# lrm2017/Fastest_Image_Pattern_Matching

Hardware: AMD Instinct MI355X
Metric: template matches/sec + ms/search, 4024×3036 src ±180°; HBM GB/s vs roofline (higher is better)
Workload: dtype u8

## Files before the change

### fastest_image_pattern_matching_amd/csrc/fpm_kernels.hip

```cpp
#include <float.h>
#include <stdio.h>
#include <stdlib.h>
#include <limits.h>

#include <map>
#include <mutex>
#include <type_traits>
#include <utility>

#include "fpm_kernels.h"
#include "fpm_rrect.h"

static void ensure_lds_attr(const void* fn, size_t bytes) {
    if (bytes <= 65536) return;
    int dev = 0;
    (void)hipGetDevice(&dev);
    static std::mutex mu;
    static std::map<std::pair<int, const void*>, size_t> done;
    std::lock_guard<std::mutex> lock(mu);
    size_t& cur = done[std::make_pair(dev, fn)];
    if (bytes <= cur) return;
    (void)hipFuncSetAttribute(fn, hipFuncAttributeMaxDynamicSharedMemorySize, (int)bytes);
    cur = bytes;
}
// ... 2523 lines not shown
                        } else {
                            pk = bilerp_row4(v, fxv, fyv);
                        }
                    }
                    if (ABL == 4 ? pk == 0x9e3779b9u && c0 < 0 : ry0 + lr + 8 * i <= ry1)
                        st_at<uint32_t>(tile, st_lane + 256u * i, (pk & colmask) ^ kRoiFlip);
                }
                continue;
            }
#pragma unroll
            for (int i = 0; i < 4; ++i) {
                if (ry0 + lr + 8 * i > ry1) break;
                uint32_t pk = 0;
#pragma unroll
                for (int u = 0; u < 4; ++u) {
                    const int X = (int)(X0r[i] + adv[u]) >> kTapShift;
                    const int Y = (int)(Y0r[i] + bdv[u]) >> kTapShift;
                    int v;
                    if (in_lds) {
                        const int sx = sat_s16(X >> kInterBits), sy = sat_s16(Y >> kInterBits);
                        const int fx = X & (kInterTab - 1), fy = Y & (kInterTab - 1);
                        const uint8_t* p = FT + (sy - by0) * ftw + (sx - bxa);
                        int v0, v1, v2, v3;
                        if ((unsigned)sx < (unsigned)(W - 1) && (unsigned)sy < (unsigned)(H - 1)) {
                            v0 = p[0]; v1 = p[1]; v2 = p[ftw]; v3 = p[ftw + 1];
                        } else if (sx >= W || sx + 1 < 0 || sy >= H || sy + 1 < 0) {
                            v0 = v1 = v2 = v3 = 0;
                        } else {
                            const bool x0 = sx >= 0 && sx < W, x1 = sx + 1 >= 0 && sx + 1 < W;
                            const bool y0 = sy >= 0 && sy < H, y1 = sy + 1 >= 0 && sy + 1 < H;
                            v0 = x0 && y0 ? p[0] : 0;
                            v1 = x1 && y0 ? p[1] : 0;
                            v2 = x0 && y1 ? p[ftw] : 0;
                            v3 = x1 && y1 ? p[ftw + 1] : 0;
                        }
                        const int h0 = 32 * v0 + fx * (v1 - v0), h1 = 32 * v2 + fx * (v3 - v2);
                        v = (32 * h0 + fy * (h1 - h0) + 512) >> 10;
                    } else {
                        v = roi_tap(lvl, W, H, a.P, X, Y);
                    }
                    if (c0 + u >= RW) v = 0;
                    pk |= (uint32_t)v << (8 * u);
                }
                st_at<uint32_t>(tile, st_lane + 256u * i, pk ^ kRoiFlip);
            }
        }
    }
}

typedef int fpm_v4i __attribute__((ext_vector_type(4)));
constexpr int kBandRows = 2 * kMmaRows;
constexpr int kBandSrc = kBandRows + 6;
constexpr int kStageRows = (kBandSrc + 3) / 4;
constexpr int kStageBatch = 5;

__device__ __forceinline__ uint32_t wave_sum_u32(uint32_t v) {
#pragma unroll
    for (int m = 32; m >= 1; m >>= 1) v += (uint32_t)__shfl_xor((int)v, m, 64);
    return v;
}

__device__ __forceinline__ uint32_t funnel(uint32_t hi, uint32_t lo, int sh) {
    return sh == 0 ? lo : __builtin_amdgcn_alignbyte(hi, lo, sh);
}

__device__ __forceinline__ void band_mfma(const uint8_t* ap, const uint8_t* bp, int nk, fpm_v4i acc[7]) {
    fpm_v4i c0 = {0, 0, 0, 0}, c1 = c0, c2 = c0, c3 = c0, c4 = c0, c5 = c0, c6 = c0;
    for (int k = 0; k < nk; ++k) {
        const fpm_v4i av = *(const fpm_v4i*)__builtin_assume_aligned(ap + 64 * k, 16);
        const uint8_t* bk = (const uint8_t*)__builtin_assume_aligned(bp + 64 * k, 16);
        const uint4 lo = *(const uint4*)bk;
        const uint2 hi = *(const uint2*)(bk + 16);
        const uint32_t w0 = lo.x, w1 = lo.y, w2 = lo.z, w3 = lo.w, w4 = hi.x, w5 = hi.y;
        const uint32_t a10 = __builtin_amdgcn_alignbyte(w1, w0, 1), a21 = __builtin_amdgcn_alignbyte(w2, w1, 1),
                       a32 = __builtin_amdgcn_alignbyte(w3, w2, 1), a43 = __builtin_amdgcn_alignbyte(w4, w3, 1),
                       a54 = __builtin_amdgcn_alignbyte(w5, w4, 1);
        const uint32_t b10 = __builtin_amdgcn_alignbyte(w1, w0, 2), b21 = __builtin_amdgcn_alignbyte(w2, w1, 2),
                       b32 = __builtin_amdgcn_alignbyte(w3, w2, 2), b43 = __builtin_amdgcn_alignbyte(w4, w3, 2),
                       b54 = __builtin_amdgcn_alignbyte(w5, w4, 2);
        const uint32_t e10 = __builtin_amdgcn_alignbyte(w1, w0, 3), e21 = __builtin_amdgcn_alignbyte(w2, w1, 3),
                       e32 = __builtin_amdgcn_alignbyte(w3, w2, 3), e43 = __builtin_amdgcn_alignbyte(w4, w3, 3);
        c0 = __builtin_amdgcn_mfma_i32_16x16x64_i8(av, fpm_v4i{(int)w0, (int)w1, (int)w2, (int)w3}, c0, 0, 0, 0);
        c1 = __builtin_amdgcn_mfma_i32_16x16x64_i8(av, fpm_v4i{(int)a10, (int)a21, (int)a32, (int)a43}, c1, 0, 0, 0);
        c2 = __builtin_amdgcn_mfma_i32_16x16x64_i8(av, fpm_v4i{(int)b10, (int)b21, (int)b32, (int)b43}, c2, 0, 0, 0);
        c3 = __builtin_amdgcn_mfma_i32_16x16x64_i8(av, fpm_v4i{(int)e10, (int)e21, (int)e32, (int)e43}, c3, 0, 0, 0);
        c4 = __builtin_amdgcn_mfma_i32_16x16x64_i8(av, fpm_v4i{(int)w1, (int)w2, (int)w3, (int)w4}, c4, 0, 0, 0);
        c5 = __builtin_amdgcn_mfma_i32_16x16x64_i8(av, fpm_v4i{(int)a21, (int)a32, (int)a43, (int)a54}, c5, 0, 0, 0);
        c6 = __builtin_amdgcn_mfma_i32_16x16x64_i8(av, fpm_v4i{(int)b21, (int)b32, (int)b43, (int)b54}, c6, 0, 0, 0);
    }
    acc[0] = c0; acc[1] = c1; acc[2] = c2; acc[3] = c3; acc[4] = c4; acc[5] = c5; acc[6] = c6;
}

__device__ __forceinline__ void band_mfma_ga(const int8_t* ap, const uint8_t* bp, int nk, fpm_v4i acc[7]) {
    fpm_v4i c0 = {0, 0, 0, 0}, c1 = c0, c2 = c0, c3 = c0, c4 = c0, c5 = c0, c6 = c0;
    fpm_v4i p0 = *(const fpm_v4i*)ap, p1 = *(const fpm_v4i*)(ap + 64);
    for (int k = 0; k < nk; ++k) {
        const fpm_v4i av = p0;
        p0 = p1;
        p1 = *(const fpm_v4i*)(ap + 64 * (k + 2));
        asm volatile("" ::: "memory");
        const uint8_t* bk = (const uint8_t*)__builtin_assume_aligned(bp + 64 * k, 16);
        const uint4 lo = *(const uint4*)bk;
        const uint2 hi = *(const uint2*)(bk + 16);
        const uint32_t w0 = lo.x, w1 = lo.y, w2 = lo.z, w3 = lo.w, w4 = hi.x, w5 = hi.y;
        const uint32_t a10 = __builtin_amdgcn_alignbyte(w1, w0, 1), a21 = __builtin_amdgcn_alignbyte(w2, w1, 1),
                       a32 = __builtin_amdgcn_alignbyte(w3, w2, 1), a43 = __builtin_amdgcn_alignbyte(w4, w3, 1),
                       a54 = __builtin_amdgcn_alignbyte(w5, w4, 1);
        const uint32_t b10 = __builtin_amdgcn_alignbyte(w1, w0, 2), b21 = __builtin_amdgcn_alignbyte(w2, w1, 2),
                       b32 = __builtin_amdgcn_alignbyte(w3, w2, 2), b43 = __builtin_amdgcn_alignbyte(w4, w3, 2),
                       b54 = __builtin_amdgcn_alignbyte(w5, w4, 2);
        const uint32_t e10 = __builtin_amdgcn_alignbyte(w1, w0, 3), e21 = __builtin_amdgcn_alignbyte(w2, w1, 3),
                       e32 = __builtin_amdgcn_alignbyte(w3, w2, 3), e43 = __builtin_amdgcn_alignbyte(w4, w3, 3);
        c0 = __builtin_amdgcn_mfma_i32_16x16x64_i8(av, fpm_v4i{(int)w0, (int)w1, (int)w2, (int)w3}, c0, 0, 0, 0);
        c1 = __builtin_amdgcn_mfma_i32_16x16x64_i8(av, fpm_v4i{(int)a10, (int)a21, (int)a32, (int)a43}, c1, 0, 0, 0);
        c2 = __builtin_amdgcn_mfma_i32_16x16x64_i8(av, fpm_v4i{(int)b10, (int)b21, (int)b32, (int)b43}, c2, 0, 0, 0);
        c3 = __builtin_amdgcn_mfma_i32_16x16x64_i8(av, fpm_v4i{(int)e10, (int)e21, (int)e32, (int)e43}, c3, 0, 0, 0);
        c4 = __builtin_amdgcn_mfma_i32_16x16x64_i8(av, fpm_v4i{(int)w1, (int)w2, (int)w3, (int)w4}, c4, 0, 0, 0);
        c5 = __builtin_amdgcn_mfma_i32_16x16x64_i8(av, fpm_v4i{(int)a21, (int)a32, (int)a43, (int)a54}, c5, 0, 0, 0);
        c6 = __builtin_amdgcn_mfma_i32_16x16x64_i8(av, fpm_v4i{(int)b21, (int)b32, (int)b43, (int)b54}, c6, 0, 0, 0);
    }
    acc[0] = c0; acc[1] = c1; acc[2] = c2; acc[3] = c3; acc[4] = c4; acc[5] = c5; acc[6] = c6;
}

template <int NK>
__device__ __forceinline__ void band_mfma_regs(const fpm_v4i* A, const uint8_t* bp, int nk, fpm_v4i acc[7]) {
    fpm_v4i c0 = {0, 0, 0, 0}, c1 = c0, c2 = c0, c3 = c0, c4 = c0, c5 = c0, c6 = c0;
#pragma unroll
    for (int k = 0; k < NK; ++k) {
        if (k >= nk) continue;
        const fpm_v4i av = A[k];
        const uint8_t* bk = (const uint8_t*)__builtin_assume_aligned(bp + 64 * k, 16);
        const uint4 lo = *(const uint4*)bk;
        const uint2 hi = *(const uint2*)(bk + 16);
        const uint32_t w0 = lo.x, w1 = lo.y, w2 = lo.z, w3 = lo.w, w4 = hi.x, w5 = hi.y;
        const uint32_t a10 = __builtin_amdgcn_alignbyte(w1, w0, 1), a21 = __builtin_amdgcn_alignbyte(w2, w1, 1),
                       a32 = __builtin_amdgcn_alignbyte(w3, w2, 1), a43 = __builtin_amdgcn_alignbyte(w4, w3, 1),
                       a54 = __builtin_amdgcn_alignbyte(w5, w4, 1);
        const uint32_t b10 = __builtin_amdgcn_alignbyte(w1, w0, 2), b21 = __builtin_amdgcn_alignbyte(w2, w1, 2),
                       b32 = __builtin_amdgcn_alignbyte(w3, w2, 2), b43 = __builtin_amdgcn_alignbyte(w4, w3, 2),
                       b54 = __builtin_amdgcn_alignbyte(w5, w4, 2);
        const uint32_t e10 = __builtin_amdgcn_alignbyte(w1, w0, 3), e21 = __builtin_amdgcn_alignbyte(w2, w1, 3),
                       e32 = __builtin_amdgcn_alignbyte(w3, w2, 3), e43 = __builtin_amdgcn_alignbyte(w4, w3, 3);
        c0 = __builtin_amdgcn_mfma_i32_16x16x64_i8(av, fpm_v4i{(int)w0, (int)w1, (int)w2, (int)w3}, c0, 0, 0, 0);
        c1 = __builtin_amdgcn_mfma_i32_16x16x64_i8(av, fpm_v4i{(int)a10, (int)a21, (int)a32, (int)a43}, c1, 0, 0, 0);
        c2 = __builtin_amdgcn_mfma_i32_16x16x64_i8(av, fpm_v4i{(int)b10, (int)b21, (int)b32, (int)b43}, c2, 0, 0, 0);
        c3 = __builtin_amdgcn_mfma_i32_16x16x64_i8(av, fpm_v4i{(int)e10, (int)e21, (int)e32, (int)e43}, c3, 0, 0, 0);
        c4 = __builtin_amdgcn_mfma_i32_16x16x64_i8(av, fpm_v4i{(int)w1, (int)w2, (int)w3, (int)w4}, c4, 0, 0, 0);
        c5 = __builtin_amdgcn_mfma_i32_16x16x64_i8(av, fpm_v4i{(int)a21, (int)a32, (int)a43, (int)a54}, c5, 0, 0, 0);
        c6 = __builtin_amdgcn_mfma_i32_16x16x64_i8(av, fpm_v4i{(int)b21, (int)b32, (int)b43, (int)b54}, c6, 0, 0, 0);
    }
    acc[0] = c0; acc[1] = c1; acc[2] = c2; acc[3] = c3; acc[4] = c4; acc[5] = c5; acc[6] = c6;
}

#ifndef FPM_CORR_PRIO
#define FPM_CORR_PRIO 1
#endif
template <int MODE, bool GA, int WPE, int NK = 0, bool PFR = true, int RS = 1, bool SE = false, bool DMA = false,
          bool DB = false>
__global__ __launch_bounds__(256) __attribute__((amdgpu_waves_per_eu(WPE))) void k_roi_corr(RoiArgs a) {
    static_assert(!DMA || (NK > 0 && !PFR), "LDS-DMA staging replaces the register staging of the register-A form");
    static_assert(!DB || DMA, "the double buffer is filled by LDS-DMA");
    static_assert(NK == 0 || (GA && MODE != 3), "the register-A form stages no template rows");
    static_assert(!SE || NK > 0, "the staged epilogue is flushed in the register-A form's staging phase");
    extern __shared__ __attribute__((aligned(16))) uint8_t smem[];
    const int tw = a.tw, th = a.th, RW = tw + 6;
    const int SBp = a.roi_pitch;
    const int TBp = tmpl_lds_pitch(a.tp8);
    uint8_t* const SB0 = smem;
    uint8_t* SB = SB0;
    uint8_t* TB = SB + (size_t)kBandSrc * SBp;
    uint32_t* rall = (uint32_t*)(TB + (GA ? 0 : (size_t)kBandRows * TBp));
    uint32_t* rallq = rall + kBandSrc;
    uint32_t* wi = rallq + kBandSrc;
    uint32_t* wq = wi + kBandSrc * 7;
    uint32_t* lts = wq + kBandSrc * 7;
    uint32_t* rsb = lts + 2 * kMmaRows;
    uint8_t* const SB1 = (uint8_t*)(((uintptr_t)(rsb + 2 * kMmaRows * 49) + 64 + 15) & ~(uintptr_t)15);
    const int tid = threadIdx.x, lane = tid & 63, wv = tid >> 6;
    const int nband = (th + kBandRows - 1) / kBandRows;
    const int rois = roi_count(a), items = rois * nband;
    const int q4 = SBp >> 4;
    const int nwr = (RW + 3) >> 2;
    const int g = lane >> 4, n = lane & 15;
    const int mt = wv & 1, nt = mt + (wv >> 1);
    const int txn = (RW + ROI_T - 1) / ROI_T;
    const XcdSplit xs = xcd_split(items);
    int it_lo = xs.lo + xs.k, it_hi = xs.hi, it_step = xs.nk;
    if (NK > 0) {
        const int64_t span = xs.hi - xs.lo;
        it_lo = xs.lo + (int)(span * xs.k / xs.nk);
        it_hi = xs.lo + (int)(span * (xs.k + 1) / xs.nk);
        it_step = 1;
    }
    constexpr int NA = NK > 0 ? NK : 1;
    fpm_v4i Areg[NA];
#pragma unroll
    for (int k = 0; k < NA; ++k) Areg[k] = fpm_v4i{0, 0, 0, 0};
    int a_band = -1;
    uint4 pv[kStageRows];
    const int lc = min(lane, 2 * txn - 1);
    auto load_rows = [&](int it) {
        const int bd = it / rois, sl = it - bd * rois;
        const int T0n = bd * kBandRows, nsn = min(kBandRows, th - T0n) + 6;
        const uint8_t* rsrc = a.roi + (size_t)sl * a.roi_stride;
        const int wvu = __builtin_amdgcn_readfirstlane(wv);
        int lcv = lc;
        asm volatile("" : "+v"(lcv));
        const uint32_t lane_off = ((uint32_t)(lcv >> 1) << 10) + 16u * (uint32_t)(lcv & 1);
#pragma unroll
        for (int i = 0; i < kStageRows; ++i) {
            const int R = T0n + min(wvu + 4 * i, nsn - 1);
            pv[i] = *(const uint4*)(rsrc + ((size_t)((R >> 5) * txn) << 10) + (R & 31) * ROI_T + lane_off);
        }
    };
    if (NK > 0 && PFR && it_lo < it_hi) load_rows(it_lo);
    int pv_slot = -1, pv_T0 = 0, pv_rb = 0;
    auto flush = [&]() {
        if (!SE || pv_slot < 0) return;
        uint32_t* dst = a.rowsum + (((size_t)th * 49 + 3) & ~(size_t)3) * pv_slot + (size_t)pv_T0 * 49;
        const int nw = pv_rb * 49, n16 = nw >> 2;
        for (int i = tid; i < n16; i += 256) *(uint4*)(dst + 4 * i) = *(const uint4*)(rsb + 4 * i);
        if (tid < (nw & 3)) dst[4 * n16 + tid] = rsb[4 * n16 + tid];
    };
    auto dma_rows = [&](int it, uint8_t* buf) {
        const int bd = it / rois, sl = it - bd * rois;
        const int T0n = bd * kBandRows, nsn = min(kBandRows, th - T0n) + 6;
        const uint8_t* rsrc = a.roi + (size_t)sl * a.roi_stride;
        const uint32_t lane_off = ((uint32_t)(lane >> 1) << 10) + 16u * (uint32_t)(lane & 1);
        const int wvu = __builtin_amdgcn_readfirstlane(wv);
        const bool in_roi = lane < 2 * txn;
#pragma unroll
        for (int i = 0; i < kStageRows; ++i) {
            const int r = wvu + 4 * i;
            if (r < nsn && in_roi) {
                const int R = T0n + r;
                const uint8_t* gp = rsrc + ((size_t)((R >> 5) * txn) << 10) + (R & 31) * ROI_T + lane_off;
                const uint32_t ldsa = __builtin_amdgcn_readfirstlane(lds_offset_of(buf + (size_t)r * SBp));
                uint32_t keep;
                asm volatile("s_mov_b32 %0, m0\n\ts_mov_b32 m0, %2\n\ts_nop 0\n\tglobal_load_lds_dwordx4 %1, off\n\t"
                             "s_mov_b32 m0, %0"
                             : "=&s"(keep) : "v"(gp), "s"(ldsa) : "memory");
            }
        }
    };
    for (int item = it_lo; item < it_hi; item += it_step) {
        int slot, band;
        if (NK > 0) { band = item / rois; slot = item - band * rois; }
        else { slot = item / nband; band = item - slot * nband; }
        SB = DB && ((item - it_lo) & 1) ? SB1 : SB0;
        const int T0 = band * kBandRows, rb = min(kBandRows, th - T0), nsrc = rb + 6;
        __syncthreads();
        if (RS == 0 && tid < kBandSrc) { rall[tid] = 0; rallq[tid] = 0; }
        if (NK > 0) {
            const bool in_roi = lane < 2 * txn;
            if (DB) {
                if (item == it_lo) dma_rows(item, SB);
                asm volatile("s_waitcnt vmcnt(0)" ::: "memory");
                flush();
            } else if (DMA) {
                dma_rows(item, SB);
                flush();
                asm volatile("s_waitcnt vmcnt(0)" ::: "memory");
            } else {
            if (!PFR) load_rows(item);
            flush();
#pragma unroll
            for (int i = 0; i < kStageRows; ++i) {
                const int r = wv + 4 * i;
                if (r < nsrc && lane < q4)
                    *(uint4*)(SB + (size_t)r * SBp + 16 * lane) = in_roi ? pv[i] : make_uint4(kRoiFlip, kRoiFlip, kRoiFlip, kRoiFlip);
            }
            }
            if (band != a_band) {
                a_band = band;
                if (tid < kBandRows) lts[tid] = tid < rb ? (uint32_t)a.tsum[T0 + tid] : 0u;
                if (kMmaRows * mt < rb) {
                    const int8_t* ap = a.tmpl8 + (size_t)(T0 + kMmaRows * mt + n) * a.tp8 + 16 * g;
#pragma unroll
                    for (int k = 0; k < NA; ++k)
                        if (k < a.nk) Areg[k] = *(const fpm_v4i*)(ap + 64 * k);
                }
            }
            if (PFR && item + 1 < it_hi) load_rows(item + 1);
        } else if (MODE != 3) {
            if (tid < kBandRows) lts[tid] = tid < rb ? (uint32_t)a.tsum[T0 + tid] : 0u;
            const uint8_t* rsrc = a.roi + (size_t)slot * a.roi_stride;
            for (int c0 = 0; c0 < q4; c0 += 64) {
                const int c = c0 + lane;
                for (int i0 = 0; i0 < kStageRows; i0 += kStageBatch) {
                    uint4 v[kStageBatch];
#pragma unroll
                    for (int i = 0; i < kStageBatch; ++i) {
                        const int r = wv + 4 * (i0 + i);
                        const int R = T0 + r;
                        v[i] = (r < nsrc && c < 2 * txn)
                                   ? *(const uint4*)(rsrc + ((size_t)((R >> 5) * txn + (c >> 1)) << 10) + (R & 31) * ROI_T + 16 * (c & 1))
                                   : make_uint4(kRoiFlip, kRoiFlip, kRoiFlip, kRoiFlip);
                    }
#pragma unroll
                    for (int i = 0; i < kStageBatch; ++i) {
                        const int r = wv + 4 * (i0 + i);
                        if (r < nsrc && c < q4) *(uint4*)(SB + (size_t)r * SBp + 16 * c) = v[i];
                    }
                }
            }
        }
        __syncthreads();
        if (DB && item + 1 < it_hi) dma_rows(item + 1, SB == SB0 ? SB1 : SB0);
        if (RS >= 1 && MODE != 7 && tid < 4 * nsrc) {
            const int r = tid >> 2, qq = tid & 3;
            const int per = (nwr + 3) >> 2, k0 = qq * per, k1 = min(nwr, k0 + per);
            const uint32_t* row = (const uint32_t*)(SB + (size_t)r * SBp);
            uint32_t s1 = 0, s2 = 0;
            int k = k0;
            for (; k + 8 <= k1; k += 8) {
                uint32_t x[8];
#pragma unroll
                for (int u = 0; u < 8; ++u) x[u] = row[k + u] ^ 0x80808080u;
#pragma unroll
                for (int u = 0; u < 8; ++u) {
                    s1 = __builtin_amdgcn_udot4(x[u], 0x01010101u, s1, false);
                    s2 = __builtin_amdgcn_udot4(x[u], x[u], s2, false);
                }
            }
            for (; k < k1; ++k) {
                const uint32_t x = row[k] ^ 0x80808080u;
                s1 = __builtin_amdgcn_udot4(x, 0x01010101u, s1, false);
                s2 = __builtin_amdgcn_udot4(x, x, s2, false);
            }
            const uint32_t l0 = row[0] ^ 0x80808080u, l1 = row[1] ^ 0x80808080u;
            const int wr = tw >> 2;
            const uint32_t x0 = row[wr], x1 = row[wr + 1], x2 = row[wr + 2];
            const uint32_t e0 = __builtin_amdgcn_alignbyte(x1, x0, (uint32_t)tw) ^ 0x80808080u;
            const uint32_t e1 = __builtin_amdgcn_alignbyte(x2, x1, (uint32_t)tw) ^ 0x80808080u;
            s1 += (uint32_t)__builtin_amdgcn_mov_dpp((int)s1, 0xB1, 0xF, 0xF, false);
            s2 += (uint32_t)__builtin_amdgcn_mov_dpp((int)s2, 0xB1, 0xF, 0xF, false);
            s1 += (uint32_t)__builtin_amdgcn_mov_dpp((int)s1, 0x4E, 0xF, 0xF, false);
            s2 += (uint32_t)__builtin_amdgcn_mov_dpp((int)s2, 0x4E, 0xF, 0xF, false);
#pragma unroll
            for (int h = 0; h < 2; ++h) {
                const int dx = qq + 4 * h;
                if (dx < 7) {
                    const uint32_t ml0 = dx >= 4 ? 0xffffffffu : (1u << (8 * dx)) - 1u;
                    const uint32_t ml1 = dx <= 4 ? 0u : (1u << (8 * (dx - 4))) - 1u;
                    const uint32_t mr0 = dx >= 4 ? 0u : ~((1u << (8 * dx)) - 1u);
                    const uint32_t mr1 = dx <= 4 ? 0xffffu : dx == 5 ? 0xff00u : 0u;
                    const uint32_t a0 = l0 & ml0, a1 = l1 & ml1, b0 = e0 & mr0, b1 = e1 & mr1;
                    uint32_t q1 = __builtin_amdgcn_udot4(a0, 0x01010101u, 0u, false);
                    q1 = __builtin_amdgcn_udot4(a1, 0x01010101u, q1, false);
                    q1 = __builtin_amdgcn_udot4(b0, 0x01010101u, q1, false);
                    q1 = __builtin_amdgcn_udot4(b1, 0x01010101u, q1, false);
                    uint32_t q2 = __builtin_amdgcn_udot4(a0, a0, 0u, false);
                    q2 = __builtin_amdgcn_udot4(a1, a1, q2, false);
                    q2 = __builtin_amdgcn_udot4(b0, b0, q2, false);
                    q2 = __builtin_amdgcn_udot4(b1, b1, q2, false);
                    wi[r * 7 + dx] = s1 - q1;
                    wq[r * 7 + dx] = s2 - q2;
                }
            }
        }
        if (RS == 0 && MODE != 7 && tid < 4 * nsrc) {
            const int r = tid >> 2, qq = tid & 3;
            const int per = (nwr + 3) >> 2, k0 = qq * per, k1 = min(nwr, k0 + per);
            const uint32_t* row = (const uint32_t*)(SB + (size_t)r * SBp);
            uint32_t s1 = 0, s2 = 0;
            int k = k0;
            for (; k + 8 <= k1; k += 8) {
                uint32_t x[8];
#pragma unroll
                for (int u = 0; u < 8; ++u) x[u] = row[k + u] ^ 0x80808080u;
#pragma unroll
                for (int u = 0; u < 8; ++u) {
                    s1 = __builtin_amdgcn_udot4(x[u], 0x01010101u, s1, false);
                    s2 = __builtin_amdgcn_udot4(x[u], x[u], s2, false);
                }
            }
            for (; k < k1; ++k) {
                const uint32_t x = row[k] ^ 0x80808080u;
                s1 = __builtin_amdgcn_udot4(x, 0x01010101u, s1, false);
                s2 = __builtin_amdgcn_udot4(x, x, s2, false);
            }
            atomicAdd(&rall[r], s1);
            atomicAdd(&rallq[r], s2);
        }
        if (!GA) {
            const int trows = (rb + kMmaRows - 1) / kMmaRows * kMmaRows;
            stage_block16(TB, TBp, (const uint8_t*)a.tmpl8 + (size_t)T0 * a.tp8, a.tp8, trows, a.tp8 >> 4, tid, 256);
        }
        if (RS == 0) __syncthreads();
        for (int i = tid; RS == 0 && MODE != 4 && i < nsrc * 7; i += 256) {
            const int r = i / 7, dx = i - r * 7;
            const uint8_t* sbr = SB + (size_t)r * SBp;
            uint32_t q1 = rall[r], q2 = rallq[r];
            for (int c = 0; c < dx; ++c) { const uint32_t v = sbr[c] ^ 0x80u; q1 -= v; q2 -= v * v; }
            for (int c = dx + tw; c < RW; ++c) { const uint32_t v = sbr[c] ^ 0x80u; q1 -= v; q2 -= v * v; }
            wi[i] = q1;
            wq[i] = q2;
        }
        __syncthreads();
        auto partials = [&]() {
            if (MODE == 6 || tid >= 4 * 49) return;
            const int pr = tid >> 1, half = tid & 1;
            const int h = pr / 49, k = pr - h * 49;
            const int chunk = (T0 >> 4) + h;
            const int tlo = kMmaRows * h, thi = min(tlo + kMmaRows, rb);
            const bool ok = chunk < a.nchunk && tlo < thi;
            const int pdy = k / 7, ddx = k - pdy * 7;
            const int t0 = tlo + 8 * half, n8 = ok ? min(8, thi - t0) : 0;
            uint32_t s1 = 0, x[8], y[8];
#pragma unroll
            for (int u = 0; u < 8; ++u) {
                const int i = (t0 + u + pdy) * 7 + ddx;
                x[u] = u < n8 ? wi[i] : 0u;
                y[u] = u < n8 ? wq[i] : 0u;
            }
            uint64_t s2 = 0;
#pragma unroll
            for (int u = 0; u < 8; ++u) { s1 += x[u]; s2 += y[u]; }
            s1 += (uint32_t)__builtin_amdgcn_mov_dpp((int)s1, 0xB1, 0xF, 0xF, false);
            const uint32_t lo = (uint32_t)s2, hi = (uint32_t)(s2 >> 32);
            s2 += (uint64_t)(uint32_t)__builtin_amdgcn_mov_dpp((int)lo, 0xB1, 0xF, 0xF, false) |
                  ((uint64_t)(uint32_t)__builtin_amdgcn_mov_dpp((int)hi, 0xB1, 0xF, 0xF, false) << 32);
            if (ok && half == 0) {
                uint32_t kk = (uint32_t)k;
                asm volatile("" : "+v"(kk));
                const uint32_t wo = ((uint32_t)slot * (uint32_t)a.nchunk + (uint32_t)chunk) * 49u + kk;
                a.wsum[wo] = s1;
                a.wsq[wo] = s2;
            }
        };
        if (RS == 2) partials();
        const bool active = kMmaRows * mt < rb && kMmaRows * nt < nsrc;
        if (FPM_CORR_PRIO == 1) __builtin_amdgcn_s_setprio(1);
        if (MODE != 2 && active) {
            int sr = kMmaRows * nt + n;
            if (sr >= nsrc) sr = 0;
            const uint8_t* bp = SB + (size_t)sr * SBp + 16 * g;
            fpm_v4i acc[7];
            if (FPM_CORR_PRIO == 2) __builtin_amdgcn_s_setprio(1);
            if (NK > 0)
                band_mfma_regs<NA>(Areg, bp, a.nk, acc);
            else if (GA)
                band_mfma_ga(a.tmpl8 + (size_t)(T0 + kMmaRows * mt + n) * a.tp8 + 16 * g, bp, a.nk, acc);
            else
                band_mfma(TB + (size_t)(kMmaRows * mt + n) * TBp + 16 * g, bp, a.nk, acc);
            if (FPM_CORR_PRIO == 2) __builtin_amdgcn_s_setprio(0);
            uint32_t* rs_out = a.rowsum + (((size_t)th * 49 + 3) & ~(size_t)3) * slot + (size_t)T0 * 49;
            const uint32_t kFix = 16384u * (uint32_t)tw;
            int t0 = kMmaRows * mt + 4 * g;
            asm volatile("" : "+v"(t0));
            const int s_ = kMmaRows * nt + n;
            const uint4 ts4 = *(const uint4*)(lts + t0);
#pragma unroll
            for (int r = 0; r < 4; ++r) {
                const int t = t0 + r, dy = s_ - t;
                if (t < rb && s_ < nsrc && dy >= 0 && dy < 7) {
                    const uint32_t ts = r == 0 ? ts4.x : r == 1 ? ts4.y : r == 2 ? ts4.z : ts4.w;
                    if (MODE == 5) {
                        uint32_t x = ts;
#pragma unroll
                        for (int d = 0; d < 7; ++d) x += (uint32_t)acc[d][r];
                        if (x == 0x9e3779b9u && a.W < 0) rs_out[t] = x;
                        continue;
                    }
                    const uint32_t o = (uint32_t)(t * 49 + dy * 7);
                    if (SE) {
#pragma unroll
                        for (int d = 0; d < 7; ++d) rsb[o + d] = (uint32_t)acc[d][r] + 128u * (wi[s_ * 7 + d] + ts) - kFix;
                        continue;
                    }
#pragma unroll
                    for (int d = 0; d < 7; ++d) rs_out[o + d] = (uint32_t)acc[d][r] + 128u * (wi[s_ * 7 + d] + ts) - kFix;
                }
            }
        }
        if (FPM_CORR_PRIO == 1) __builtin_amdgcn_s_setprio(0);
        if (RS == 1) partials();
        if (RS == 0 && MODE != 6 && tid < 2 * 49) {
            const int h = tid / 49, k = tid - h * 49;
            const int chunk = (T0 >> 4) + h;
            const int tlo = kMmaRows * h, thi = min(tlo + kMmaRows, rb);
            if (chunk < a.nchunk && tlo < thi) {
                const int pdy = k / 7, ddx = k - pdy * 7;
                uint32_t s1 = 0;
                uint64_t s2 = 0;
                for (int t = tlo; t < thi; ++t) {
                    s1 += wi[(t + pdy) * 7 + ddx];
                    s2 += wq[(t + pdy) * 7 + ddx];
                }
                a.wsum[((size_t)slot * a.nchunk + chunk) * 49 + k] = s1;
                a.wsq[((size_t)slot * a.nchunk + chunk) * 49 + k] = s2;
            }
        }
        if (SE) { pv_slot = slot; pv_T0 = T0; pv_rb = rb; }
    }
    if (SE && pv_slot >= 0) {
        __syncthreads();
        flush();
    }
}

#ifdef FPM_EXPERIMENTAL
constexpr int kB16Rows = kMmaRows, kB16Src = kB16Rows + 6;
__host__ __device__ inline size_t roi_corr16_lds(int roi_pitch) {
    return (size_t)kB16Src * roi_pitch + sizeof(uint32_t) * (2 * 7 * kB16Src + kB16Rows + kB16Rows * 49) + 64;
}
template <int NK, int WPE>
__global__ __launch_bounds__(128) __attribute__((amdgpu_waves_per_eu(WPE))) void k_roi_corr16(RoiArgs a) {
    extern __shared__ __attribute__((aligned(16))) uint8_t smem[];
    constexpr int NT = 128;
    const int tw = a.tw, th = a.th, RW = tw + 6;
    const int SBp = a.roi_pitch;
    uint8_t* const SB = smem;
    uint32_t* wi = (uint32_t*)(SB + (size_t)kB16Src * SBp);
    uint32_t* wq = wi + kB16Src * 7;
    uint32_t* lts = wq + kB16Src * 7;
    uint32_t* rsb = lts + kB16Rows;
    const int tid = threadIdx.x, lane = tid & 63, wv = tid >> 6;
    const int nband = (th + kB16Rows - 1) / kB16Rows;
    const int rois = roi_count(a), items = rois * nband;
    const int nwr = (RW + 3) >> 2;
    const int g = lane >> 4, n = lane & 15;
    const int txn = (RW + ROI_T - 1) / ROI_T;
    const XcdSplit xs = xcd_split(items);
    const int64_t span = xs.hi - xs.lo;
    const int it_lo = xs.lo + (int)(span * xs.k / xs.nk), it_hi = xs.lo + (int)(span * (xs.k + 1) / xs.nk);
    fpm_v4i Areg[NK];
#pragma unroll
    for (int k = 0; k < NK; ++k) Areg[k] = fpm_v4i{0, 0, 0, 0};
    int a_band = -1;
    int pv_slot = -1, pv_T0 = 0, pv_rb = 0;
    auto flush = [&]() {
        if (pv_slot < 0) return;
        uint32_t* dst = a.rowsum + (((size_t)th * 49 + 3) & ~(size_t)3) * pv_slot + (size_t)pv_T0 * 49;
        const int nw = pv_rb * 49, n16 = nw >> 2;
        for (int i = tid; i < n16; i += NT) *(uint4*)(dst + 4 * i) = *(const uint4*)(rsb + 4 * i);
        if (tid < (nw & 3)) dst[4 * n16 + tid] = rsb[4 * n16 + tid];
    };
    auto dma_rows = [&](int it) {
        const int bd = it / rois, sl = it - bd * rois;
        const int T0n = bd * kB16Rows, nsn = min(kB16Rows, th - T0n) + 6;
        const uint8_t* rsrc = a.roi + (size_t)sl * a.roi_stride;
        const uint32_t lane_off = ((uint32_t)(lane >> 1) << 10) + 16u * (uint32_t)(lane & 1);
        const int wvu = __builtin_amdgcn_readfirstlane(wv);
        const bool in_roi = lane < 2 * txn;
#pragma unroll
        for (int i = 0; i < (kB16Src + 1) / 2; ++i) {
            const int r = wvu + 2 * i;
            if (r < nsn && in_roi) {
                const int R = T0n + r;
                const uint8_t* gp = rsrc + ((size_t)((R >> 5) * txn) << 10) + (R & 31) * ROI_T + lane_off;
                const uint32_t ldsa = __builtin_amdgcn_readfirstlane(lds_offset_of(SB + (size_t)r * SBp));
                uint32_t keep;
                asm volatile("s_mov_b32 %0, m0\n\ts_mov_b32 m0, %2\n\ts_nop 0\n\tglobal_load_lds_dwordx4 %1, off\n\t"
                             "s_mov_b32 m0, %0"
                             : "=&s"(keep) : "v"(gp), "s"(ldsa) : "memory");
            }
        }
    };
    for (int item = it_lo; item < it_hi; ++item) {
        const int band = item / rois, slot = item - band * rois;
        const int T0 = band * kB16Rows, rb = min(kB16Rows, th - T0), nsrc = rb + 6;
        __syncthreads();
        dma_rows(item);
        flush();
        asm volatile("s_waitcnt vmcnt(0)" ::: "memory");
        if (band != a_band) {
            a_band = band;
            if (tid < kB16Rows) lts[tid] = tid < rb ? (uint32_t)a.tsum[T0 + tid] : 0u;
            const int8_t* ap = a.tmpl8 + (size_t)(T0 + n) * a.tp8 + 16 * g;
#pragma unroll
            for (int k = 0; k < NK; ++k)
                if (k < a.nk) Areg[k] = *(const fpm_v4i*)(ap + 64 * k);
        }
        __syncthreads();
        if (tid < 4 * nsrc) {
            const int r = tid >> 2, qq = tid & 3;
            const int per = (nwr + 3) >> 2, k0 = qq * per, k1 = min(nwr, k0 + per);
            const uint32_t* row = (const uint32_t*)(SB + (size_t)r * SBp);
            uint32_t s1 = 0, s2 = 0;
            int k = k0;
            for (; k + 8 <= k1; k += 8) {
                uint32_t x[8];
#pragma unroll
                for (int u = 0; u < 8; ++u) x[u] = row[k + u] ^ 0x80808080u;
#pragma unroll
                for (int u = 0; u < 8; ++u) {
                    s1 = __builtin_amdgcn_udot4(x[u], 0x01010101u, s1, false);
                    s2 = __builtin_amdgcn_udot4(x[u], x[u], s2, false);
                }
            }
            for (; k < k1; ++k) {
                const uint32_t x = row[k] ^ 0x80808080u;
                s1 = __builtin_amdgcn_udot4(x, 0x01010101u, s1, false);
                s2 = __builtin_amdgcn_udot4(x, x, s2, false);
            }
            const uint32_t l0 = row[0] ^ 0x80808080u, l1 = row[1] ^ 0x80808080u;
            const int wr = tw >> 2;
            const uint32_t x0 = row[wr], x1 = row[wr + 1], x2 = row[wr + 2];
            const uint32_t e0 = __builtin_amdgcn_alignbyte(x1, x0, (uint32_t)tw) ^ 0x80808080u;
            const uint32_t e1 = __builtin_amdgcn_alignbyte(x2, x1, (uint32_t)tw) ^ 0x80808080u;
            s1 += (uint32_t)__builtin_amdgcn_mov_dpp((int)s1, 0xB1, 0xF, 0xF, false);
            s2 += (uint32_t)__builtin_amdgcn_mov_dpp((int)s2, 0xB1, 0xF, 0xF, false);
            s1 += (uint32_t)__builtin_amdgcn_mov_dpp((int)s1, 0x4E, 0xF, 0xF, false);
            s2 += (uint32_t)__builtin_amdgcn_mov_dpp((int)s2, 0x4E, 0xF, 0xF, false);
#pragma unroll
            for (int h = 0; h < 2; ++h) {
                const int dx = qq + 4 * h;
                if (dx < 7) {
                    const uint32_t ml0 = dx >= 4 ? 0xffffffffu : (1u << (8 * dx)) - 1u;
                    const uint32_t ml1 = dx <= 4 ? 0u : (1u << (8 * (dx - 4))) - 1u;
                    const uint32_t mr0 = dx >= 4 ? 0u : ~((1u << (8 * dx)) - 1u);
                    const uint32_t mr1 = dx <= 4 ? 0xffffu : dx == 5 ? 0xff00u : 0u;
                    const uint32_t a0 = l0 & ml0, a1 = l1 & ml1, b0 = e0 & mr0, b1 = e1 & mr1;
                    uint32_t q1 = __builtin_amdgcn_udot4(a0, 0x01010101u, 0u, false);
                    q1 = __builtin_amdgcn_udot4(a1, 0x01010101u, q1, false);
                    q1 = __builtin_amdgcn_udot4(b0, 0x01010101u, q1, false);
                    q1 = __builtin_amdgcn_udot4(b1, 0x01010101u, q1, false);
                    uint32_t q2 = __builtin_amdgcn_udot4(a0, a0, 0u, false);
                    q2 = __builtin_amdgcn_udot4(a1, a1, q2, false);
                    q2 = __builtin_amdgcn_udot4(b0, b0, q2, false);
                    q2 = __builtin_amdgcn_udot4(b1, b1, q2, false);
                    wi[r * 7 + dx] = s1 - q1;
                    wq[r * 7 + dx] = s2 - q2;
                }
            }
        }
        __syncthreads();
        if (kMmaRows * wv < nsrc) {
            int sr = kMmaRows * wv + n;
// ... 800 lines not shown
            for (int u = 0; u < 8; ++u) { x[u] = ws[(size_t)(c + u) * 49]; y[u] = wq[(size_t)(c + u) * 49]; }
#pragma unroll
            for (int u = 0; u < 8; ++u) { s1 += x[u]; s2 += y[u]; }
        }
        for (; c < a.nchunk; ++c) { s1 += ws[(size_t)c * 49]; s2 += wq[(size_t)c * 49]; }
    }
    constexpr int BQ = kEvalRows * 49 / 4;
    const int nblk = (th + kEvalRows - 1) / kEvalRows;
    auto issue_block = [&](int b, uint8_t* buf) {
#pragma unroll
        for (int i = 0; i < kEvalDma; ++i) {
            size_t q = (size_t)b * BQ + 64 * i + lane;
            if (64 * i + lane >= BQ || q >= total4) q = 0;
            uint32_t keep;
            const uint32_t ldsa = (uint32_t)(uintptr_t)(fpm_lds_vp)(buf + 1024 * i);
            asm volatile("s_mov_b32 %0, m0\n\ts_mov_b32 m0, %2\n\ts_nop 0\n\tglobal_load_lds_dwordx4 %1, off\n\ts_mov_b32 m0, %0"
                         : "=&s"(keep) : "v"(rs + q), "s"(__builtin_amdgcn_readfirstlane(ldsa)) : "memory");
        }
    };
    float accF = 0.f;
    uint64_t accI = 0;
    issue_block(0, blk);
    for (int b = 0; b < nblk; ++b) {
        const uint32_t* cb = (const uint32_t*)(blk + (b & 1) * kEvalBuf);
        if (b + 1 < nblk) {
            issue_block(b + 1, blk + ((b + 1) & 1) * kEvalBuf);
            asm volatile("s_waitcnt vmcnt(%0)" :: "i"(kEvalDma) : "memory");
        } else {
            asm volatile("s_waitcnt vmcnt(0)" ::: "memory");
        }
        wave_sync();
        const int rows = min(kEvalRows, th - b * kEvalRows);
        if (lane < 49) {
            if (a.fold) {
                int t = 0;
                for (; t + 8 <= rows; t += 8) {
                    uint32_t x[8];
#pragma unroll
                    for (int u = 0; u < 8; ++u) x[u] = cb[(t + u) * 49 + lane];
#pragma unroll
                    for (int u = 0; u < 8; ++u) accF = accF + (float)(int)x[u];
                }
                for (; t < rows; ++t) accF = accF + (float)(int)cb[t * 49 + lane];
            } else {
                for (int t = 0; t < rows; ++t) accI += cb[t * 49 + lane];
            }
        }
        wave_sync();
    }
    if (lane < 49) {
        const double num = a.fold ? (double)accF : (double)(float)(double)accI;
        sc[lane] = ccoeff(num, (double)s1, (double)s2, a.mean, a.norm, a.inv_area);
    }
    wave_sync();
    if (lane == 0) {
        float best = sc[0];
        int bi = 0;
        for (int k = 1; k < 49; ++k)
            if (sc[k] > best) { best = sc[k]; bi = k; }
        const int mx = bi % 7, my = bi / 7;
        RoiRecord r;
        r.score = best;
        r.mx = (int16_t)mx;
        r.my = (int16_t)my;
        const int border = (mx == 0 || my == 0 || mx == 6 || my == 6) ? 1 : 0;
        r.on_border = border;
        for (int x = -1; x <= 1; ++x)
            for (int y = -1; y <= 1; ++y) r.vec[(x + 1) * 3 + (y + 1)] = border ? 0.f : sc[(my + y) * 7 + (mx + x)];
        *out = r;
        *keep = r;
    }
}

template <int ROWS>
__global__ __launch_bounds__(192) void k_roi_eval(RoiArgs a) {
    __shared__ __attribute__((aligned(16))) uint8_t blk_all[3][2 * EvalBlk<ROWS>::buf];
    __shared__ float sc_all[3][64];
    __shared__ RoiRecord recs[3];
    __shared__ int pos;
    __shared__ CandState ns;
    __shared__ AngleNode nn[3];
    const int lane = threadIdx.x & 63, j = threadIdx.x >> 6;
    const int rois = roi_count(a);
    const int base = roi_base(a);
    const int c_lo = base / a.n3, c_hi = (base + rois) / a.n3;
    for (int li = c_lo + blockIdx.x; li < c_hi; li += gridDim.x) {
        const int id = a.live[li];
        const int slot = li * a.n3 + j - base;
        __syncthreads();
        eval_roi<ROWS>(a, slot, lane, blk_all[j], sc_all[j], a.rec + (size_t)id * a.n3 + j, &recs[j]);
        if (!a.step) continue;
        __syncthreads();
        if (threadIdx.x == 0) {
            float score[3];
            int mx[3], my[3];
            for (int k = 0; k < a.n3; ++k) { score[k] = recs[k].score; mx[k] = recs[k].mx; my[k] = recs[k].my; }
            CandState s;
            pos = cand_step_one(a, id, score, mx, my, &s, a.nt_tab ? nn : nullptr);
            ns = s;
        }
        if (!a.nt_tab) continue;
        __syncthreads();
        if (pos >= 0) cand_next_tables(a, id, pos, ns, nn[j], j, lane);
    }
}

void launch_roi_tables(const RoiArgs& a, hipStream_t st) {
    if (a.slot_cap <= 0 || a.equal1) return;
    const int grid = a.slot_cap < 4096 ? a.slot_cap : 4096;
    hipLaunchKernelGGL(k_roi_tables, dim3(grid), dim3(256), 0, st, a);
}

constexpr int kWarpFootBatch = 12, kWarpWaves = 8;
static int grid_cap_env(const char* v, int dflt) { return v ? (atoi(v) > 0 ? atoi(v) : 0) : dflt; }
static int capped(int grid, int cap) { return cap > 0 && grid > cap ? cap : grid; }
static int device_cus() {
    int dev = 0;
    (void)hipGetDevice(&dev);
    static std::mutex mu;
    static std::map<int, int> cus;
    std::lock_guard<std::mutex> lock(mu);
    auto it = cus.find(dev);
    if (it != cus.end()) return it->second;
    int n = 0;
    if (hipDeviceGetAttribute(&n, hipDeviceAttributeMultiprocessorCount, dev) != hipSuccess || n <= 0) n = 256;
    cus[dev] = n;
    return n;
}
void launch_roi_warp(const RoiArgs& a, hipStream_t st) {
    if (a.slot_cap <= 0 || a.equal1) return;
    const long tiles = (long)a.slot_cap * ((a.th + 6 + ROI_T - 1) / ROI_T) * ((a.tw + 6 + ROI_T - 1) / ROI_T);
    if (tiles > INT_MAX) return;
    const long want = (tiles + 3) / 4;
    const int grid = (int)(want < 16384 ? want : 16384);
    const char* w3e = getenv("FPM_WARP3");
    const int warp3 = w3e ? atoi(w3e) : 1;
    if (warp3 && a.n3 == 3 && a.slot_base % 3 == 0 && a.slot_cap % 3 == 0) {
        const long want3 = (tiles / 3 + 3) / 4;
        const int srcs = a.slot_cap / std::max(1, a.per_source * a.n3);
        const int dflt_cap = srcs <= 2 ? 7 * device_cus() : 0;
        hipLaunchKernelGGL((k_roi_warp3<7, kFtPitch, 0>), dim3(capped((int)(want3 < 16384 ? want3 : 16384), grid_cap_env(getenv("FPM_GRID_WARP"), dflt_cap))),
                           dim3(256), 0, st, a);
        return;
    }
    hipLaunchKernelGGL((k_roi_warp<kWarpFootBatch, 0, kWarpWaves>), dim3(grid), dim3(256), 0, st, a);
}

constexpr size_t kLdsPerCu = 160 * 1024;
constexpr bool kCorrGlobalA = true;
constexpr int kCorrWaves = 3;
constexpr int kCorrRunWaves = 2;
template <int NK>
static void launch_corr_regs(const RoiArgs& a, long items, size_t lds, hipStream_t st) {
    if constexpr (NK <= 12) {
        if (NK == 4 && lds * 4 <= kLdsPerCu) {
            const int grid = capped((int)std::min<long>(items, 4L * device_cus()), grid_cap_env(getenv("FPM_GRID_CORR"), 0));
            hipLaunchKernelGGL((k_roi_corr<0, true, 4, NK, false, 1, true>), dim3(grid), dim3(256), lds, st, a);
            return;
        }
        if ((NK == 8 || NK == 12) && lds * 4 <= kLdsPerCu) {
            const int grid = capped((int)std::min<long>(items, 4L * device_cus()), grid_cap_env(getenv("FPM_GRID_CORR"), 0));
            hipLaunchKernelGGL((k_roi_corr<0, true, 4, NK, false, 1, true, true>), dim3(grid), dim3(256), lds, st, a);
            return;
        }
        const int grid = capped((int)std::min<long>(items, (long)kCorrWaves * device_cus()), grid_cap_env(getenv("FPM_GRID_CORR"), 0));
        hipLaunchKernelGGL((k_roi_corr<0, true, kCorrWaves, NK, false, 1, true>), dim3(grid), dim3(256), lds, st, a);
    } else {
        const int grid = (int)std::min<long>(items, (long)kCorrRunWaves * device_cus());
        hipLaunchKernelGGL((k_roi_corr<0, true, kCorrRunWaves, NK>), dim3(grid), dim3(256), lds, st, a);
    }
}
#ifdef FPM_EXPERIMENTAL
bool launch_roi_corr16(const RoiArgs& a, hipStream_t st) {
    if (a.nk > 12 || (a.roi_pitch >> 4) > 64) return false;
    const size_t lds = roi_corr16_lds(a.roi_pitch);
    const int per_cu = (int)std::min<size_t>(8, kLdsPerCu / lds);
    if (per_cu < 1) return false;
    const long items = (long)a.slot_cap * ((a.th + kB16Rows - 1) / kB16Rows);
    const int grid = capped((int)std::min<long>(items, (long)per_cu * device_cus()), grid_cap_env(getenv("FPM_GRID_CORR"), 0));
    if (a.nk <= 4) hipLaunchKernelGGL((k_roi_corr16<4, 4>), dim3(grid), dim3(128), lds, st, a);
    else if (a.nk <= 8) hipLaunchKernelGGL((k_roi_corr16<8, 4>), dim3(grid), dim3(128), lds, st, a);
    else hipLaunchKernelGGL((k_roi_corr16<12, 4>), dim3(grid), dim3(128), lds, st, a);
    return true;
}

#endif

void launch_roi_corr(const RoiArgs& a, hipStream_t st) {
    if (a.slot_cap <= 0 || a.equal1) return;
    const size_t lds = roi_corr_lds(a.roi_pitch, a.tw, a.rc, kCorrGlobalA);
    if ((a.roi_pitch >> 4) <= 64 && a.nk <= 16 && lds <= 65536) {
        const long items = (long)a.slot_cap * ((a.th + kBandRows - 1) / kBandRows);
        if (a.nk <= 4) launch_corr_regs<4>(a, items, lds, st);
        else if (a.nk <= 8) launch_corr_regs<8>(a, items, lds, st);
        else if (a.nk <= 12) launch_corr_regs<12>(a, items, lds, st);
        else launch_corr_regs<16>(a, items, lds, st);
        return;
    }
    ensure_lds_attr((const void*)k_roi_corr<0, kCorrGlobalA, kCorrWaves>, lds);
    const long items = (long)a.slot_cap * ((a.th + kBandRows - 1) / kBandRows);
    const int grid = (int)(items < 16384 ? items : 16384);
    hipLaunchKernelGGL((k_roi_corr<0, kCorrGlobalA, kCorrWaves>), dim3(grid), dim3(256), lds, st, a);
}

#ifdef FPM_EXPERIMENTAL
void launch_roi_fused(const RoiArgs& a, hipStream_t st) {
    if (a.slot_cap <= 0 || a.equal1) return;
    const size_t lds = (size_t)fuse_layout(a.tw).total;
    const long units = (long)a.slot_cap * a.nparts;
    const int grid = (int)(units < kFuseWgs ? units : kFuseWgs);
    if (a.nk <= 4) hipLaunchKernelGGL(k_roi_fused<4>, dim3(grid), dim3(256), lds, st, a);
    else if (a.nk <= 8) hipLaunchKernelGGL(k_roi_fused<8>, dim3(grid), dim3(256), lds, st, a);
    else if (a.nk <= 12) hipLaunchKernelGGL(k_roi_fused<12>, dim3(grid), dim3(256), lds, st, a);
    else hipLaunchKernelGGL(k_roi_fused<16>, dim3(grid), dim3(256), lds, st, a);
}
#endif

void launch_roi_eval(const RoiArgs& a, hipStream_t st) {
    if (a.slot_cap <= 0) return;
    const int cands = (a.slot_cap + a.n3 - 1) / a.n3;
    const int grid = cands < 4096 ? cands : 4096;
    const int srcs = a.slot_cap / std::max(1, a.per_source * a.n3);
    if (srcs <= 2) hipLaunchKernelGGL(k_roi_eval<48>, dim3(grid), dim3(64 * a.n3), 0, st, a);
    else hipLaunchKernelGGL(k_roi_eval<40>, dim3(grid), dim3(64 * a.n3), 0, st, a);
}

void launch_roi_small(const RoiArgs& a, hipStream_t st) {
    if (a.slot_cap <= 0) return;
    if (a.equal1) {
        RoiArgs b = a;
        b.step = 0;
        launch_roi_eval(b, st);
        return;
    }
    const char* nte = getenv("FPM_SMALL_NT");
    const int srcs = a.slot_cap / std::max(1, a.per_source * a.n3);
    const int kCUs = device_cus();
    if (nte ? atoi(nte) == 512 : (srcs <= 2 && a.slot_cap <= 4 * kCUs)) {
        const size_t lds8 = (size_t)small_layout(a.tw, a.th, 8).total;
        const int grid = capped(a.slot_cap < 8192 ? a.slot_cap : 8192, grid_cap_env(getenv("FPM_GRID_SMALL"), kCUs));
        if (a.prev_rec) {
            ensure_lds_attr((const void*)k_roi_small<0, 2, true, 512>, lds8);
            hipLaunchKernelGGL((k_roi_small<0, 2, true, 512>), dim3(grid), dim3(512), lds8, st, a);
        } else {
            ensure_lds_attr((const void*)k_roi_small<0, 2, false, 512>, lds8);
            hipLaunchKernelGGL((k_roi_small<0, 2, false, 512>), dim3(grid), dim3(512), lds8, st, a);
        }
        return;
    }
    const size_t lds2 = (size_t)small_layout(a.tw, a.th, 2).total, lds4 = (size_t)small_layout(a.tw, a.th).total;
    const int per_cu2 = (int)std::min<size_t>(8, kLdsPerCu / std::max<size_t>(lds2, 1));
    const int per_cu4 = (int)std::min<size_t>((size_t)(lds4 * 4 <= kLdsPerCu ? 4 : 3), kLdsPerCu / std::max<size_t>(lds4, 1));
    const int nt_env = nte ? atoi(nte) : 0;
    if (!a.prev_rec && a.tw + 6 <= 512 && per_cu2 > per_cu4 && nt_env != 256 &&
        (nt_env == 128 || a.slot_cap > per_cu4 * kCUs)) {
        const int grid = capped(a.slot_cap < 16384 ? a.slot_cap : 16384,
                                grid_cap_env(getenv("FPM_GRID_SMALL"), per_cu2 * kCUs));
        ensure_lds_attr((const void*)k_roi_small<0, 4, false, 128>, lds2);
        hipLaunchKernelGGL((k_roi_small<0, 4, false, 128>), dim3(grid), dim3(128), lds2, st, a);
        return;
    }
    const size_t lds = lds4;
    const int wpe = a.prev_rec ? 3 : (lds * 4 <= kLdsPerCu ? 4 : 3);
    const int per_cu = (int)std::min<size_t>((size_t)wpe, kLdsPerCu / std::max<size_t>(lds, 1));
    const int grid = capped(a.slot_cap < 8192 ? a.slot_cap : 8192,
                            grid_cap_env(getenv("FPM_GRID_SMALL"), std::max(per_cu, 1) * kCUs));
    if (a.prev_rec) {
        ensure_lds_attr((const void*)k_roi_small<0, 3, true>, lds);
        hipLaunchKernelGGL((k_roi_small<0, 3, true>), dim3(grid), dim3(256), lds, st, a);
        return;
    }
    if (lds * 4 <= kLdsPerCu) {
        ensure_lds_attr((const void*)k_roi_small<0, 4>, lds);
        hipLaunchKernelGGL((k_roi_small<0, 4>), dim3(grid), dim3(256), lds, st, a);
        return;
    }
    ensure_lds_attr((const void*)k_roi_small<0>, lds);
    hipLaunchKernelGGL(k_roi_small<0>, dim3(grid), dim3(256), lds, st, a);
}

void launch_cand_step(const RoiArgs& a, int max_items, hipStream_t st) {
    if (max_items <= 0 || !a.step) return;
    if (a.nt_tab) {
        const int grid = max_items < 2048 ? max_items : 2048;
        hipLaunchKernelGGL(k_cand_step_tab, dim3(grid), dim3(192), 0, st, a);
        return;
    }
    int grid = (max_items + 255) / 256;
    if (grid > 1024) grid = 1024;
    hipLaunchKernelGGL(k_cand_step, dim3(grid), dim3(256), 0, st, a);
}

constexpr int TM_BH = 16;
constexpr int TM_CP2 = 224, TM_CP1 = 288;
constexpr int TM_FTP = 44;
constexpr int TM_FTB = 44 * 40;
#ifndef TOPMMA_ABL
#define TOPMMA_ABL 0
#endif
#ifndef TOPMMA_PRIO
#define TOPMMA_PRIO 4
#endif

bool top_mma_fits(int tw, int th) { return tw >= 1 && th >= 1 && ((tw <= 17 && th <= 32) || (tw <= 49 && th <= 16)); }

static bool top_mma_small(const TopMmaArgs& a) { return a.R == 2 && a.th <= 16; }

void top_mma_layout(TopMmaArgs& a, int sw, int max_rows) {
    a.sw = sw;
    a.R = a.tw <= 17 ? 2 : 1;
    a.nq = a.R == 2 ? (a.th + 1) / 2 : a.th;
    a.cp = top_mma_small(a) ? TM_CP2 : TM_CP1;
    a.rr = top_mma_small(a) ? 32 : 64;
    a.ct = (sw + a.tw - 1 + 8 + 3) & ~3;
    a.rt = max_rows + a.th;
    a.o_colt = 3 * a.rr * a.cp;
    a.o_rowt = a.o_colt + 8 * a.ct;
    a.o_bf = (a.o_rowt + 8 * a.rt + 15) & ~15;
    a.nqm = top_mma_small(a) ? 8 : 16;
    a.o_ft = a.o_bf + 1024 * a.nqm;
}
size_t top_mma_lds(const TopMmaArgs& a) { return (size_t)a.o_ft + 4 * TM_FTB; }
// ... 472 lines not shown
```

Baseline: 35590.

## Compute window row sums with matrix-core MFMA and dot4 edge corrections

Adds new row-sum modes (RS 3/4) to the ROI correlation kernel. Per-row sums and sums of squares over the template width are computed with i8 MFMA (a ones-vector for sums, self-products for squares) or sdot4, with a signed-offset correction. Each of the 7 shifted windows is then derived by subtracting the edge bytes with udot4. The padding bytes are pre-filled so every staged byte is defined. This replaces the old scalar per-thread row-sum loop, at the cost of extra MFMA work, padding writes and a cross-lane shuffle.

```diff
diff --git a/fastest_image_pattern_matching_amd/csrc/fpm_kernels.hip b/fastest_image_pattern_matching_amd/csrc/fpm_kernels.hip
--- a/fastest_image_pattern_matching_amd/csrc/fpm_kernels.hip
+++ b/fastest_image_pattern_matching_amd/csrc/fpm_kernels.hip
@@ -2699,6 +2699,77 @@
     acc[0] = c0; acc[1] = c1; acc[2] = c2; acc[3] = c3; acc[4] = c4; acc[5] = c5; acc[6] = c6;
 }
 
+template <bool VS = false>
+__device__ __forceinline__ void tile_row_sums(const uint8_t* bp, int nk, int n, uint32_t& s1, uint32_t& s2) {
+    const fpm_v4i ones = {0x01010101, 0x01010101, 0x01010101, 0x01010101};
+    fpm_v4i cs = {0, 0, 0, 0}, cq = cs;
+    int vs = 0;
+    auto dot16 = [](fpm_v4i b, int acc) {
+        acc = __builtin_amdgcn_sdot4(b[0], 0x01010101, acc, false);
+        acc = __builtin_amdgcn_sdot4(b[1], 0x01010101, acc, false);
+        acc = __builtin_amdgcn_sdot4(b[2], 0x01010101, acc, false);
+        return __builtin_amdgcn_sdot4(b[3], 0x01010101, acc, false);
+    };
+    int k = 0;
+    for (; k + 4 <= nk; k += 4) {
+        fpm_v4i b[4];
+#pragma unroll
+        for (int u = 0; u < 4; ++u) b[u] = *(const fpm_v4i*)__builtin_assume_aligned(bp + 64 * (k + u), 16);
+#pragma unroll
+        for (int u = 0; u < 4; ++u) {
+            if (VS) vs = dot16(b[u], vs); else cs = __builtin_amdgcn_mfma_i32_16x16x64_i8(ones, b[u], cs, 0, 0, 0);
+            cq = __builtin_amdgcn_mfma_i32_16x16x64_i8(b[u], b[u], cq, 0, 0, 0);
+        }
+    }
+    if (k + 2 <= nk) {
+        const fpm_v4i b0 = *(const fpm_v4i*)__builtin_assume_aligned(bp + 64 * k, 16);
+        const fpm_v4i b1 = *(const fpm_v4i*)__builtin_assume_aligned(bp + 64 * k + 64, 16);
+        if (VS) vs = dot16(b0, vs); else cs = __builtin_amdgcn_mfma_i32_16x16x64_i8(ones, b0, cs, 0, 0, 0);
+        cq = __builtin_amdgcn_mfma_i32_16x16x64_i8(b0, b0, cq, 0, 0, 0);
+        if (VS) vs = dot16(b1, vs); else cs = __builtin_amdgcn_mfma_i32_16x16x64_i8(ones, b1, cs, 0, 0, 0);
+        cq = __builtin_amdgcn_mfma_i32_16x16x64_i8(b1, b1, cq, 0, 0, 0);
+        k += 2;
+    }
+    if (k < nk) {
+        const fpm_v4i b0 = *(const fpm_v4i*)__builtin_assume_aligned(bp + 64 * k, 16);
+        if (VS) vs = dot16(b0, vs); else cs = __builtin_amdgcn_mfma_i32_16x16x64_i8(ones, b0, cs, 0, 0, 0);
+        cq = __builtin_amdgcn_mfma_i32_16x16x64_i8(b0, b0, cq, 0, 0, 0);
+    }
+    const int e = n & 3;
+    if (VS) {
+        vs += __shfl_xor(vs, 16, 64);
+        vs += __shfl_xor(vs, 32, 64);
+    }
+    const uint32_t p1 = (uint32_t)(VS ? vs : cs[0]);
+    const uint32_t p2 = (uint32_t)(e == 0 ? cq[0] : e == 1 ? cq[1] : e == 2 ? cq[2] : cq[3]);
+    const uint32_t C = 64u * (uint32_t)nk;
+    s1 = p1 + 128u * C;
+    s2 = p2 + 256u * p1 + 16384u * C;
+}
+
+__device__ __forceinline__ void window_edges(uint64_t lo, uint64_t hi, int dx, int nf, uint32_t& q1, uint32_t& q2) {
+    const uint64_t ldx = (1ull << (8 * dx)) - 1ull, lnf = (1ull << (8 * nf)) - 1ull;
+    const uint64_t sl = lo & ldx;
+    const uint64_t sr = hi & lnf & ~ldx;
+    const uint64_t ar = hi & ldx & ~lnf;
+    const uint32_t a0 = (uint32_t)sl, a1 = (uint32_t)(sl >> 32), b0 = (uint32_t)sr, b1 = (uint32_t)(sr >> 32);
+    const uint32_t c0 = (uint32_t)ar, c1 = (uint32_t)(ar >> 32);
+    uint32_t p1 = __builtin_amdgcn_udot4(a0, 0x01010101u, 0u, false);
+    p1 = __builtin_amdgcn_udot4(a1, 0x01010101u, p1, false);
+    p1 = __builtin_amdgcn_udot4(b0, 0x01010101u, p1, false);
+    p1 = __builtin_amdgcn_udot4(b1, 0x01010101u, p1, false);
+    uint32_t m1 = __builtin_amdgcn_udot4(c0, 0x01010101u, 0u, false);
+    m1 = __builtin_amdgcn_udot4(c1, 0x01010101u, m1, false);
+    uint32_t p2 = __builtin_amdgcn_udot4(a0, a0, 0u, false);
+    p2 = __builtin_amdgcn_udot4(a1, a1, p2, false);
+    p2 = __builtin_amdgcn_udot4(b0, b0, p2, false);
+    p2 = __builtin_amdgcn_udot4(b1, b1, p2, false);
+    uint32_t m2 = __builtin_amdgcn_udot4(c0, c0, 0u, false);
+    m2 = __builtin_amdgcn_udot4(c1, c1, m2, false);
+    q1 = p1 - m1;
+    q2 = p2 - m2;
+}
+
 #ifndef FPM_CORR_PRIO
 #define FPM_CORR_PRIO 1
 #endif
@@ -2709,6 +2780,7 @@
     static_assert(!DB || DMA, "the double buffer is filled by LDS-DMA");
     static_assert(NK == 0 || (GA && MODE != 3), "the register-A form stages no template rows");
     static_assert(!SE || NK > 0, "the staged epilogue is flushed in the register-A form's staging phase");
+    static_assert(RS < 3 || NK > 0, "the matrix-core row sums read the register-A form's staged rows, every byte defined");
     extern __shared__ __attribute__((aligned(16))) uint8_t smem[];
     const int tw = a.tw, th = a.th, RW = tw + 6;
     const int SBp = a.roi_pitch;
@@ -2731,6 +2803,7 @@
     const int g = lane >> 4, n = lane & 15;
     const int mt = wv & 1, nt = mt + (wv >> 1);
     const int txn = (RW + ROI_T - 1) / ROI_T;
+    const int npad = max(0, (min(ROI_T * txn, 64 * a.nk) - 4 * nwr) >> 2);
     const XcdSplit xs = xcd_split(items);
     int it_lo = xs.lo + xs.k, it_hi = xs.hi, it_step = xs.nk;
     if (NK > 0) {
@@ -2761,6 +2834,14 @@
         }
     };
     if (NK > 0 && PFR && it_lo < it_hi) load_rows(it_lo);
+    if (RS >= 3 && DMA) {
+        const int nfill = q4 - 2 * txn;
+        for (int b = 0; b < (DB ? 2 : 1); ++b)
+            for (int i = tid; i < kBandSrc * nfill; i += 256) {
+                const int r = i / nfill, c = 2 * txn + (i - r * nfill);
+                *(uint4*)((b ? SB1 : SB0) + (size_t)r * SBp + 16 * c) = make_uint4(kRoiFlip, kRoiFlip, kRoiFlip, kRoiFlip);
+            }
+    }
     int pv_slot = -1, pv_T0 = 0, pv_rb = 0;
     auto flush = [&]() {
         if (!SE || pv_slot < 0) return;
@@ -2854,7 +2935,38 @@
         }
         __syncthreads();
         if (DB && item + 1 < it_hi) dma_rows(item + 1, SB == SB0 ? SB1 : SB0);
-        if (RS >= 1 && MODE != 7 && tid < 4 * nsrc) {
+        if (RS >= 3 && MODE != 7 && wv != 2 && kMmaRows * nt < nsrc) {
+            int ln = lane;
+            asm volatile("" : "+v"(ln));
+            const int g3 = ln >> 4, n3 = ln & 15, row = kMmaRows * nt + n3;
+            const int sr = row < nsrc ? row : 0;
+            uint32_t* rw = (uint32_t*)(SB + (size_t)sr * SBp);
+            if (npad > 0) {
+                if (g3 < npad) rw[nwr + g3] = kRoiFlip;
+                if (g3 + 4 < npad) rw[nwr + g3 + 4] = kRoiFlip;
+            }
+            const int wr = tw >> 2;
+            const uint32_t l0 = rw[0], l1 = rw[1], x0 = rw[wr], x1 = rw[wr + 1], x2 = rw[wr + 2];
+            uint32_t s1, s2;
+            tile_row_sums<RS == 4>((const uint8_t*)rw + 16 * g3, a.nk, n3, s1, s2);
+            s2 = (uint32_t)__shfl((int)s2, n3 + 16 * (n3 >> 2), 64);
+            const uint32_t e0 = __builtin_amdgcn_alignbyte(x1, x0, (uint32_t)tw) ^ 0x80808080u;
+            const uint32_t e1 = __builtin_amdgcn_alignbyte(x2, x1, (uint32_t)tw) ^ 0x80808080u;
+            const uint64_t lo = (uint64_t)(l0 ^ 0x80808080u) | ((uint64_t)(l1 ^ 0x80808080u) << 32);
+            const uint64_t hi = (uint64_t)e0 | ((uint64_t)e1 << 32);
+            const int nf = min(6, 64 * a.nk - tw);
+#pragma unroll
+            for (int h = 0; h < 2; ++h) {
+                const int dx = g3 + 4 * h;
+                if (dx < 7 && row < nsrc) {
+                    uint32_t q1, q2;
+                    window_edges(lo, hi, dx, nf, q1, q2);
+                    wi[row * 7 + dx] = s1 - q1;
+                    wq[row * 7 + dx] = s2 - q2;
+                }
+            }
+        }
+        if ((RS == 1 || RS == 2) && MODE != 7 && tid < 4 * nsrc) {
             const int r = tid >> 2, qq = tid & 3;
             const int per = (nwr + 3) >> 2, k0 = qq * per, k1 = min(nwr, k0 + per);
             const uint32_t* row = (const uint32_t*)(SB + (size_t)r * SBp);
@@ -3022,7 +3134,7 @@
             }
         }
         if (FPM_CORR_PRIO == 1) __builtin_amdgcn_s_setprio(0);
-        if (RS == 1) partials();
+        if (RS == 1 || RS >= 3) partials();
         if (RS == 0 && MODE != 6 && tid < 2 * 49) {
             const int h = tid / 49, k = tid - h * 49;
             const int chunk = (T0 >> 4) + h;
@@ -4129,22 +4241,23 @@
 constexpr int kCorrRunWaves = 2;
 template <int NK>
 static void launch_corr_regs(const RoiArgs& a, long items, size_t lds, hipStream_t st) {
+    constexpr int kRS = NK > 8 ? 4 : 3;
     if constexpr (NK <= 12) {
         if (NK == 4 && lds * 4 <= kLdsPerCu) {
             const int grid = capped((int)std::min<long>(items, 4L * device_cus()), grid_cap_env(getenv("FPM_GRID_CORR"), 0));
-            hipLaunchKernelGGL((k_roi_corr<0, true, 4, NK, false, 1, true>), dim3(grid), dim3(256), lds, st, a);
+            hipLaunchKernelGGL((k_roi_corr<0, true, 4, NK, false, kRS, true>), dim3(grid), dim3(256), lds, st, a);
             return;
         }
         if ((NK == 8 || NK == 12) && lds * 4 <= kLdsPerCu) {
             const int grid = capped((int)std::min<long>(items, 4L * device_cus()), grid_cap_env(getenv("FPM_GRID_CORR"), 0));
-            hipLaunchKernelGGL((k_roi_corr<0, true, 4, NK, false, 1, true, true>), dim3(grid), dim3(256), lds, st, a);
+            hipLaunchKernelGGL((k_roi_corr<0, true, 4, NK, false, kRS, true, true>), dim3(grid), dim3(256), lds, st, a);
             return;
         }
         const int grid = capped((int)std::min<long>(items, (long)kCorrWaves * device_cus()), grid_cap_env(getenv("FPM_GRID_CORR"), 0));
-        hipLaunchKernelGGL((k_roi_corr<0, true, kCorrWaves, NK, false, 1, true>), dim3(grid), dim3(256), lds, st, a);
+        hipLaunchKernelGGL((k_roi_corr<0, true, kCorrWaves, NK, false, kRS, true>), dim3(grid), dim3(256), lds, st, a);
     } else {
         const int grid = (int)std::min<long>(items, (long)kCorrRunWaves * device_cus());
-        hipLaunchKernelGGL((k_roi_corr<0, true, kCorrRunWaves, NK>), dim3(grid), dim3(256), lds, st, a);
+        hipLaunchKernelGGL((k_roi_corr<0, true, kCorrRunWaves, NK, true, kRS>), dim3(grid), dim3(256), lds, st, a);
     }
 }
 #ifdef FPM_EXPERIMENTAL
```

After: 36430, median of 6. 1.02x the previous value.
